# peter-nebe/stair-step-detector

Measured on AMD Instinct MI355X. Metric: point-cloud frames/sec (1024×768 pts) at 1/2/4/8 GPUs; step height/corner max-abs err, higher is better.
Workload: dtype f64; 1 GPU; BASELINE configs[2]: batch of 1024 synthetic 1024x768 frames (3-step staircases, randomised rise/tread/yaw/noise) resident in HBM, streamed through the whole per-frame path; per GPU; width=1024, height=768, input=float3, risers=False, batches_in_flight=3, parallelism=frame-sharded x1, no collective

## Files before the change

stair-step-detector_amd/csrc/ssd_kernels.hip:

```cpp
#ifndef SSD_CAMERAS_TU
#define SSD_ENTRY(bounds, kernel, block) __global__ bounds void kernel
#define SSD_BYVAL(T) T
#else
#define SSD_ENTRY(bounds, kernel, block) __device__ __forceinline__ void block
#define SSD_BYVAL(T) const T &
#undef SSD_PHASE_TIMING
#undef SSD_COUNT
#endif
#include "ssd_device.h"
#include "ssd_math.h"
#include "ssd_quadtest.h"
#include "ssd_closing.h"
#include "ssd_bestline.h"
#include "ssd_sort.h"

namespace ssd
{

#include "ssd_phase.h"

#ifdef SSD_CHECKED
__device__ __noinline__ void ssd_chk_report(int site, unsigned long long idx, unsigned long long limit)
{
  printf("SSD_CHECK site %d index %llu limit %llu block (%u, %u) thread %u\n", site, idx, limit, blockIdx.x, blockIdx.y, threadIdx.x);
// ... 113 lines not shown
  if(SRC == kSrcF3Aligned && idx0 + kPts <= end)
  {
    const float4 *q = reinterpret_cast<const float4 *>(base + 3 * static_cast<size_t>(idx0));
    const float4 a = q[0], b = q[1], c = q[2];
    v[0] = F3{ a.x, a.y, a.z };
    v[1] = F3{ a.w, b.x, b.y };
    v[2] = F3{ b.z, b.w, c.x };
    v[3] = F3{ c.y, c.z, c.w };
    return;
  }
#pragma unroll
  for(int j = 0; j < kPts; j++)
  {
    const int idx = idx0 + j;
    v[j] = F3{ 0.0f, 0.0f, 0.0f };
    if(idx < end)
      v[j] = *reinterpret_cast<const F3 *>(base + 3 * static_cast<size_t>(idx));
  }
}

template<int SRC>
__device__ __forceinline__ void load_points_full(const float *__restrict__ base, int idx0, F3 (&v)[kPts])
{
  if(SRC == kSrcDepth16)
    return;
  if(SRC == kSrcF3Aligned)
  {
    const float4 *q = reinterpret_cast<const float4 *>(base + 3 * static_cast<size_t>(idx0));
#ifdef SSD_NT_LOADS
    typedef float f4v __attribute__((ext_vector_type(4)));
    const f4v *qv = reinterpret_cast<const f4v *>(q);
    const f4v av = __builtin_nontemporal_load(qv), bv = __builtin_nontemporal_load(qv + 1), cv = __builtin_nontemporal_load(qv + 2);
    const float4 a = make_float4(av.x, av.y, av.z, av.w), b = make_float4(bv.x, bv.y, bv.z, bv.w), c = make_float4(cv.x, cv.y, cv.z, cv.w);
#else
    const float4 a = q[0], b = q[1], c = q[2];
#endif
    v[0] = F3{ a.x, a.y, a.z };
    v[1] = F3{ a.w, b.x, b.y };
    v[2] = F3{ b.z, b.w, c.x };
    v[3] = F3{ c.y, c.z, c.w };
    return;
  }
#pragma unroll
  for(int j = 0; j < kPts; j++)
    v[j] = *reinterpret_cast<const F3 *>(base + 3 * static_cast<size_t>(idx0 + j));
}

template<int SRC>
__device__ __forceinline__ void load_points_clamped(const float *__restrict__ base, int idx0, int end, F3 (&v)[kPts])
{
  if(SRC == kSrcDepth16)
    return;
  if(SRC == kSrcF3Aligned)
  {
    load_points_full<SRC>(base, min(idx0, end - kPts), v);
    return;
  }
#pragma unroll
  for(int j = 0; j < kPts; j++)
    v[j] = *reinterpret_cast<const F3 *>(base + 3 * static_cast<size_t>(min(idx0 + j, end - 1)));
}
__device__ __forceinline__ void zero_beyond(F3 (&v)[kPts], int idx0, int end)
{
#pragma unroll
  for(int j = 0; j < kPts; j++)
    if(idx0 + j >= end)
      v[j] = F3{ 0.0f, 0.0f, 0.0f };
}

__device__ __forceinline__ void first_use(F3 (&v)[kPts])
{
  asm volatile("" : "+v"(v[0].x), "+v"(v[0].y), "+v"(v[0].z), "+v"(v[1].x), "+v"(v[1].y), "+v"(v[1].z),
                    "+v"(v[2].x), "+v"(v[2].y), "+v"(v[2].z), "+v"(v[3].x), "+v"(v[3].y), "+v"(v[3].z));
}

#define SSD_STREAM_LOOP(body)                                                                       \
  {                                                                                                 \
    F3 va[kPts], vb[kPts];                                                                          \
    const int fullEnd = begin + (end - begin) / kTile * kTile;   \
    if(begin < fullEnd)                                                                             \
      load_points_full<SRC>(base, begin + kPts * tid, va);                                          \
    for(int i0 = begin; i0 < fullEnd; i0 += 2 * kTile)                                              \
    {                                                                                               \
      const bool more1 = i0 + kTile < fullEnd;                                                      \
      if(more1)                                                                                     \
        load_points_full<SRC>(base, i0 + kTile + kPts * tid, vb);                                   \
      body(va);                                                                                     \
      if(!more1)                                                                                    \
        break;                                                                                      \
      first_use(vb);                                                                                \
      const bool more2 = i0 + 2 * kTile < fullEnd;                                                  \
      if(more2)                                                                                     \
        load_points_full<SRC>(base, i0 + 2 * kTile + kPts * tid, va);                               \
      body(vb);                                                                                     \
      if(more2)                                                                                     \
        first_use(va);                                                                              \
    }                                                                                               \
    if(fullEnd < end)                                                                               \
    {                                                                                               \
      load_points<SRC>(base, fullEnd + kPts * tid, end, va, D);        \
      body(va);                                                                                     \
    }                                                                                               \
  }

constexpr int kBinsPerGroup = 4;
constexpr int kWavesPerBlock = kThreads / 64;
constexpr int kCell = 64;
constexpr int kCellsPerTile = kTile / kCell;
#ifndef SSD_MAX_TILES
#define SSD_MAX_TILES 32
#endif
constexpr int kMaxTilesPerBlock = SSD_MAX_TILES;
constexpr int kMaxCellsPerBlock = kMaxTilesPerBlock * kCellsPerTile;
constexpr int kMaxTilesPerBlockRaster = 128;
constexpr int kMaxCellsPerBlockRaster = kMaxTilesPerBlockRaster * kCellsPerTile;
constexpr int kMaxTilesPerBlockInquad = 128;
constexpr int kMaxCellsPerBlockInquad = kMaxTilesPerBlockInquad * kCellsPerTile;

__device__ __forceinline__ unsigned int row_or_u32(unsigned int v)
{
  v |= static_cast<unsigned int>(__builtin_amdgcn_update_dpp(0, static_cast<int>(v), 0x128, 0xf, 0xf, false));
  v |= static_cast<unsigned int>(__builtin_amdgcn_update_dpp(0, static_cast<int>(v), 0x124, 0xf, 0xf, false));
  v |= static_cast<unsigned int>(__builtin_amdgcn_update_dpp(0, static_cast<int>(v), 0x122, 0xf, 0xf, false));
  v |= static_cast<unsigned int>(__builtin_amdgcn_update_dpp(0, static_cast<int>(v), 0x121, 0xf, 0xf, false));
  return v;
}

__device__ __forceinline__ unsigned int row_min_u32(unsigned int v)
{
  v = min(v, static_cast<unsigned int>(__builtin_amdgcn_update_dpp(0, static_cast<int>(v), 0x128, 0xf, 0xf, false)));
  v = min(v, static_cast<unsigned int>(__builtin_amdgcn_update_dpp(0, static_cast<int>(v), 0x124, 0xf, 0xf, false)));
  v = min(v, static_cast<unsigned int>(__builtin_amdgcn_update_dpp(0, static_cast<int>(v), 0x122, 0xf, 0xf, false)));
  v = min(v, static_cast<unsigned int>(__builtin_amdgcn_update_dpp(0, static_cast<int>(v), 0x121, 0xf, 0xf, false)));
  return v;
}
__device__ __forceinline__ unsigned int row_max_u32(unsigned int v)
{
  v = max(v, static_cast<unsigned int>(__builtin_amdgcn_update_dpp(0, static_cast<int>(v), 0x128, 0xf, 0xf, false)));
  v = max(v, static_cast<unsigned int>(__builtin_amdgcn_update_dpp(0, static_cast<int>(v), 0x124, 0xf, 0xf, false)));
  v = max(v, static_cast<unsigned int>(__builtin_amdgcn_update_dpp(0, static_cast<int>(v), 0x122, 0xf, 0xf, false)));
  v = max(v, static_cast<unsigned int>(__builtin_amdgcn_update_dpp(0, static_cast<int>(v), 0x121, 0xf, 0xf, false)));
  return v;
}
__device__ __forceinline__ unsigned int cell_box_from_high_dwords(unsigned int x0, unsigned int x1, unsigned int y0, unsigned int y1,
                                                                  double boxX, double boxY)
{
  const unsigned int cx0 = static_cast<unsigned int>(__hiloint2double(static_cast<int>(x0), 0) * boxX);
  const unsigned int cy0 = static_cast<unsigned int>(__hiloint2double(static_cast<int>(y0), 0) * boxY);
  const unsigned int cx1 = min(static_cast<unsigned int>(__hiloint2double(static_cast<int>(x1 + 1u), 0) * boxX), 255u);
  const unsigned int cy1 = min(static_cast<unsigned int>(__hiloint2double(static_cast<int>(y1 + 1u), 0) * boxY), 255u);
  return (cx0 | (cx1 << 8)) | ((cy0 | (cy1 << 8)) << 16);
}

template<typename Want>
__device__ __forceinline__ int cell_list_build(const uint2 *__restrict__ cellInfo, int nCells, int cols, Want wantCell,
                                               unsigned short *list, unsigned int *scratch)
{
  const int tid = threadIdx.x, lane = tid & 63, wave = tid >> 6;
  const int rows = (nCells + cols - 1) / cols;
  constexpr int kFastPasses = 2;
  if(rows * cols <= kFastPasses * kThreads)
  {
    int cidx[kFastPasses];
    uint2 rec[kFastPasses];
#pragma unroll
    for(int p = 0; p < kFastPasses; p++)
    {
      const int i = p * kThreads + tid;
      const int cx = i / rows, r = i - cx * rows;
      const int c = r * cols + cx;
      cidx[p] = (cx < cols && c < nCells) ? c : -1;
      rec[p] = cidx[p] >= 0 ? cellInfo[c] : make_uint2(0u, 0u);
    }
    bool want[kFastPasses];
    int pos[kFastPasses];
#pragma unroll
    for(int p = 0; p < kFastPasses; p++)
    {
      want[p] = cidx[p] >= 0 && wantCell(rec[p]);
      const unsigned long long b = __ballot(want[p]);
      pos[p] = __popcll(b & ((1ull << lane) - 1ull));
      if(lane == 0)
        scratch[p * kWavesPerBlock + wave] = static_cast<unsigned int>(__popcll(b));
    }
    __syncthreads();
    int total = 0;
#pragma unroll
    for(int p = 0; p < kFastPasses; p++)
    {
      int before = total;
#pragma unroll
      for(int w = 0; w < kWavesPerBlock; w++)
      {
        const int n = static_cast<int>(scratch[p * kWavesPerBlock + w]);
        before += w < wave ? n : 0;
        total += n;
      }
      if(want[p])
        list[before + pos[p]] = static_cast<unsigned short>(cidx[p]);
    }
    __syncthreads();
    return total;
  }
  int total = 0;
  for(int i0 = 0; i0 < rows * cols; i0 += kThreads)
  {
    const int i = i0 + tid;
    const int cx = i / rows, r = i - cx * rows;
    const int c = r * cols + cx;
    const bool want = cx < cols && c < nCells && wantCell(cellInfo[c]);
    const unsigned long long b = __ballot(want);
    if(lane == 0)
      scratch[wave] = static_cast<unsigned int>(__popcll(b));
    __syncthreads();
    int before = total;
#pragma unroll
    for(int w = 0; w < kWavesPerBlock; w++)
    {
      const int n = static_cast<int>(scratch[w]);
      before += w < wave ? n : 0;
      total += n;
    }
    if(want)
      list[before + __popcll(b & ((1ull << lane) - 1ull))] = static_cast<unsigned short>(c);
    __syncthreads();
  }
  return total;
}

template<int SRC>
__device__ __forceinline__ void load_cell(const float *__restrict__ base, int cell0, const unsigned short *list, int entry, int count,
                                          int lane, int nPoints, F3 (&v)[kPts], const DepthSrc &D)
{
  if(entry < count)
    load_points<SRC>(base, (cell0 + static_cast<int>(list[entry])) * kCell + kPts * (lane & 15), nPoints, v, D);
  else
  {
#pragma unroll
    for(int j = 0; j < kPts; j++)
      v[j] = F3{ 0.0f, 0.0f, 0.0f };
  }
}


constexpr int kWinWords = 256;

struct ImageBox { int yMin, yMax, xMin, xMax; };

struct WaveWindow
{
  int slot = -1, row0 = 0, col0 = 0;
  unsigned int limitWords = 0xffffffffu;
};

constexpr int kWaveMissWords = 8;
__device__ __forceinline__ void wavemiss_init(unsigned int *wm)
{
  wm[0] = 0xffffffffu; wm[1] = 0u;
  wm[2] = 0x7fffffffu; wm[3] = 0xffffffffu;
  wm[4] = 0x7fffffffu; wm[5] = 0xffffffffu;
  wm[6] = 0u; wm[7] = 0u;
}
__device__ __forceinline__ void wavemiss_flush(unsigned int *wm, ImageBox *boxes, int lane)
{
  const unsigned int slots = wm[6];
  if(lane < 32 && ((slots >> lane) & 1u))
  {
    const int *b = reinterpret_cast<const int *>(wm);
    atomicMin(&boxes[lane].yMin, b[2]); atomicMax(&boxes[lane].yMax, b[3]);
    atomicMin(&boxes[lane].xMin, b[4]); atomicMax(&boxes[lane].xMax, b[5]);
  }
}

__device__ __forceinline__ int wave_min_i(int v)
{
  v = min(v, __builtin_amdgcn_update_dpp(0x7fffffff, v, 0x128, 0xf, 0xf, false));
  v = min(v, __builtin_amdgcn_update_dpp(0x7fffffff, v, 0x124, 0xf, 0xf, false));
  v = min(v, __builtin_amdgcn_update_dpp(0x7fffffff, v, 0x122, 0xf, 0xf, false));
  v = min(v, __builtin_amdgcn_update_dpp(0x7fffffff, v, 0x121, 0xf, 0xf, false));
  return min(min(__builtin_amdgcn_readlane(v, 0), __builtin_amdgcn_readlane(v, 16)), min(__builtin_amdgcn_readlane(v, 32), __builtin_amdgcn_readlane(v, 48)));
}
__device__ __forceinline__ int wave_max_i(int v)
{
  v = max(v, __builtin_amdgcn_update_dpp(static_cast<int>(0x80000000u), v, 0x128, 0xf, 0xf, false));
  v = max(v, __builtin_amdgcn_update_dpp(static_cast<int>(0x80000000u), v, 0x124, 0xf, 0xf, false));
  v = max(v, __builtin_amdgcn_update_dpp(static_cast<int>(0x80000000u), v, 0x122, 0xf, 0xf, false));
  v = max(v, __builtin_amdgcn_update_dpp(static_cast<int>(0x80000000u), v, 0x121, 0xf, 0xf, false));
  return max(max(__builtin_amdgcn_readlane(v, 0), __builtin_amdgcn_readlane(v, 16)), max(__builtin_amdgcn_readlane(v, 32), __builtin_amdgcn_readlane(v, 48)));
}

__device__ __forceinline__ void wavewin_flush(unsigned long long *ww, const WaveWindow &w, unsigned long long *__restrict__ images,
                                              unsigned int imgWords, int W64, int winShift, ImageBox *boxes, int lane)
{
  if(w.slot < 0)
    return;
  unsigned long long *img = images + static_cast<size_t>(w.slot) * imgWords;
  int y0 = 0x7fffffff, y1 = -1, x0 = 0x7fffffff, x1 = -1;
#pragma unroll
  for(int k = 0; k < kWinWords / 64; k++)
  {
    const int i = k * 64 + lane;
    const unsigned long long v = ww[i];
    if(v)
    {
      const int y = w.row0 + (i >> winShift), x = w.col0 + (i & ((1 << winShift) - 1));
      if(SSD_CHK(1, static_cast<size_t>(w.slot) * imgWords + static_cast<size_t>(y) * W64 + x, w.limitWords) && SSD_CHK(2, x, W64))
        atomicOr(img + static_cast<size_t>(y) * W64 + x, v);
      ww[i] = 0ull;
      y0 = min(y0, y); y1 = max(y1, y);
      x0 = min(x0, x); x1 = max(x1, x);
    }
  }
  y1 = wave_max_i(y1);
  if(y1 >= 0)
  {
    y0 = wave_min_i(y0); x0 = wave_min_i(x0); x1 = wave_max_i(x1);
    if(lane == 0)
    {
      atomicMin(&boxes[w.slot].yMin, y0); atomicMax(&boxes[w.slot].yMax, y1);
      atomicMin(&boxes[w.slot].xMin, x0); atomicMax(&boxes[w.slot].xMax, x1);
    }
  }
}

constexpr unsigned int kNoPixel = 0xffffffffu;
__device__ __forceinline__ unsigned int pixel_key(int slot, int iy, int ix)
{
  return (static_cast<unsigned int>(slot) << 26) | (static_cast<unsigned int>(iy) << 13) | static_cast<unsigned int>(ix);
}

__device__ __forceinline__ unsigned int wave_min_u32(unsigned int v)
{
  v = row_min_u32(v);
  return min(min(static_cast<unsigned int>(__builtin_amdgcn_readlane(static_cast<int>(v), 0)), static_cast<unsigned int>(__builtin_amdgcn_readlane(static_cast<int>(v), 16))),
             min(static_cast<unsigned int>(__builtin_amdgcn_readlane(static_cast<int>(v), 32)), static_cast<unsigned int>(__builtin_amdgcn_readlane(static_cast<int>(v), 48))));
}

constexpr unsigned int kNoWindow = 0x80000000u;
__device__ __forceinline__ unsigned int window_base(const WaveWindow &w)
{
  return w.slot < 0 ? kNoWindow : pixel_key(w.slot, w.row0, w.col0 << 6);
}
__device__ __forceinline__ bool window_hit(unsigned int d, int winShift)
{
  const unsigned int inside = (((static_cast<unsigned int>(kWinWords) >> winShift) - 1u) << 13) | ((64u << winShift) - 1u);
  return (d & ~inside) == 0u;
}

__device__ __forceinline__ void wavewin_prepare(unsigned long long *ww, WaveWindow &w, unsigned long long *__restrict__ images,
                                                unsigned int imgWords, int W64, int winShift, ImageBox *boxes, unsigned int first, int lane)
{
  const bool has = first != kNoPixel;
  const bool miss = has && !window_hit(first - window_base(w), winShift);
  const unsigned long long missing = __ballot(miss);
  if(missing == 0ull || 2 * __popcll(missing) <= __popcll(__ballot(has)))
    return;
  const unsigned int lowest = __builtin_amdgcn_readfirstlane(wave_min_u32(miss ? first : kNoPixel));
  wavewin_flush(ww, w, images, imgWords, W64, winShift, boxes, lane);
  w.slot = static_cast<int>(lowest >> 26);
  w.row0 = static_cast<int>((lowest >> 13) & 0x1fffu);
  w.col0 = max(0, min(static_cast<int>((lowest & 0x1fffu) >> 6) - 1, W64 - (1 << winShift)));
}

__device__ __forceinline__ void wavewin_emit(unsigned long long *ww, unsigned int *wm, WaveWindow &w, unsigned long long *__restrict__ images,
                                             unsigned int imgWords, int W64, int winShift, ImageBox *boxes, const unsigned int (&key)[4], int lane)
{
  wavewin_prepare(ww, w, images, imgWords, W64, winShift, boxes, min(min(key[0], key[1]), min(key[2], key[3])), lane);
  const unsigned int base = window_base(w);
  unsigned int *ww32 = reinterpret_cast<unsigned int *>(ww);
#pragma unroll
  for(int j = 0; j < 4; j++)
  {
    const unsigned int k = key[j], d = k - base;
    const unsigned int bit = 1u << (k & 31u);
    if(window_hit(d, winShift))
    {
      if(SSD_CHK(3, ((d >> 13) << (winShift + 1)) + ((d & 0x1fffu) >> 5), 2 * kWinWords))
        atomicOr(&ww32[((d >> 13) << (winShift + 1)) + ((d & 0x1fffu) >> 5)], bit);
    }
    else if(k != kNoPixel)
// ... 2028 lines not shown
    QuadTest t;
    SSD_PHASE_IF(lane == firstValid, 1, 3);
    build_quad_test(quad, t);
    err = t.err;
    SSD_PHASE_IF(lane == firstValid, 1, 4);
    const bool threwHere = __ballot(err != 0) != 0ull;
    const unsigned long long liveMask = threwHere ? 0ull : __ballot(true);
    if(!threwHere)
    {
      const int slot = __popcll(liveMask & ((1ull << lane) - 1ull));
      if(slot < kMaxLive)
      {
        fs.qtLive[slot] = t;
        QuadGridSegs sg;
        build_grid_segs(t, P.pt.xMin, P.pt.yMin, P.pt.boxX, P.pt.boxY, sg);
        fs.segLive[slot] = sg;
        QuadEdgesD w;
        quad_edges_coeffs(t, sg.ok, P.pt.xMin, P.pt.xMax, P.pt.yMin, P.pt.yMax, w, ef);
        sT[slot] = t;
        sW[slot] = w;
        sBad[slot] = 0u;
        mySlot = slot;
        fs.liveBox[slot] = live_box_thresholds(t, groundLane, P.pt);
        fs.liveAcc[slot] = static_cast<unsigned char>(lane);
        const PlateauState &pl = fs.pl[groundLane ? groundInd : lane];
        unsigned int groups = 0u;
        const int effLo = pl.effLo, effHi = pl.effHi;
        for(int b = effLo; b <= effHi; b++)
          groups |= 1u << (b / kBinsPerGroup);
        fs.liveGroups[slot] = groups;
      }
    }
  }
  {
    const int nL = __popcll(__ballot(mySlot >= 0));
    __syncthreads();
    for(int item = lane; item < nL * 9; item += 64)
    {
      const int sl = item / 9, cell = item - 9 * sl;
      if(sW[sl].fine != 0 && quad_cell_unsound(sT[sl], sW[sl], cell / 3, cell % 3))
        atomicOr(&sBad[sl], 1u);
    }
    __syncthreads();
    if(mySlot >= 0)
    {
      ef.m = quad_edges_margin(sW[mySlot], sBad[mySlot] != 0u);
      fs.edgeLive[mySlot] = ef;
    }
  }
  SSD_PHASE_IF(lane == firstValid, 1, 5);
  const bool threw = __ballot(err != 0) != 0ull;
  const bool active = (groundLane || valid) && !threw;
  if(lane <= kMaxPlateaus)
    fs.accActive[lane] = active ? 1 : 0;
  const unsigned long long activeMask = __ballot(active);
  for(int b = lane; b < kMaxBins; b += 64)
  {
    const int p = b < P.nBins ? fs.lut[b] : 0xff;
    const int acc = p == groundInd ? kGroundAcc : p;
    const bool live = p != 0xff && ((activeMask >> acc) & 1ull);
    fs.lutLive[b] = live ? static_cast<unsigned char>(__popcll(activeMask & ((1ull << acc) - 1ull))) : static_cast<unsigned char>(0xff);
  }

  SSD_PHASE_IF(lane == firstValid, 1, 6);
  unsigned int wanted = 0u;
  for(int b = lane; b < P.nBins; b += 64)
  {
    const int p = fs.lut[b];
    if(p != 0xff && ((activeMask >> (p == groundInd ? kGroundAcc : p)) & 1ull))
      wanted |= 1u << (b / kBinsPerGroup);
  }
#pragma unroll
  for(int o = 32; o > 0; o >>= 1)
    wanted |= __shfl_xor(wanted, o);
  if(lane == 0)
  {
    fs.firstValidInd = firstValid;
    if(threw)
      fs.status |= SSD_ST_THROW;
    fs.wantedQuads = wanted;
    fs.anyActive = activeMask != 0ull ? 1u : 0u;
    fs.nLive = min(__popcll(activeMask), kMaxLive);
  }
  SSD_PHASE_IF(lane == firstValid, 1, 7);
  if(dbg)
  {
    ssd_debug_frame &d = dbg[frame].d;
    if(lane == 0)
      d.first_valid_ind = firstValid;
    if(lane == kGroundAcc)
    {
      for(int k = 0; k < 8; k++)
        d.ground_quad_world[k] = groundLane ? fs.groundQuadWorld[k] : 0.0;
      d.ground_quad_err = groundLane ? err : 0;
    }
    if(lane >= first && lane < last && lane < kMaxPlateaus)
      d.plateaus[lane].quad_err = valid ? err : 0;
  }
}


constexpr int kGroundScanStep = 50;
__device__ __forceinline__ int ground_scan_x0(int W) { return (W / 2) % kGroundScanStep; }
__device__ __forceinline__ int ground_strip_row0(int H) { return H / 2 - 1; }
constexpr unsigned int strip_div50(unsigned int u) { return (u * 5243u) >> 18; }
constexpr bool strip_div50_exact()
{
  for(unsigned int u = 0; u < 16384u; u++)
    if(strip_div50(u) != u / 50u)
      return false;
  return true;
}
static_assert(strip_div50_exact(), "strip_div50 must equal u / 50 for every pixel column of an image up to 8192 wide");
__device__ __forceinline__ bool ground_strip_column(int ix, int x0)
{
  const unsigned int u = static_cast<unsigned int>(ix + 2 - x0 + kGroundScanStep);
  const unsigned int r = u - kGroundScanStep * strip_div50(u);
  return r <= 4u;
}
__device__ __forceinline__ bool ground_strip_of(int ix, int x0, int &strip, bool &centre)
{
  const unsigned int u = static_cast<unsigned int>(ix + 2 - x0 + kGroundScanStep);
  const unsigned int q = strip_div50(u), r = u - kGroundScanStep * q;
  strip = static_cast<int>(q);
  centre = r == 2u;
  return r <= 4u;
}
static_assert((8191 + 2 + kGroundScanStep) / kGroundScanStep < kMaxGroundStrips, "a strip number for every pixel column");

template<bool FULL>
struct InquadLds
{
  unsigned long long wins[FULL ? kThreads / 64 : 1][FULL ? kWinWords : 1];
  unsigned int wmiss[FULL ? kThreads / 64 : 1][kWaveMissWords];
  ImageBox box[1];
  QuadTest qts[kMaxLive];
  QuadGridSegs segs[kMaxLive];
  QuadEdgesF edges[kMaxLive + 1];
  K1Consts kc;
  unsigned char lut[kMaxBins];
  unsigned long long lsum[kMaxLive][8];
  unsigned int lcnt[kMaxLive][8];
  unsigned int lOob;
  unsigned short cellList[kMaxCellsPerBlockInquad];
  unsigned int listScratch[2 * kWavesPerBlock];
  unsigned int liveGroups[kMaxLive];
  int4 liveBox[kMaxLive];
  unsigned char liveAcc[kMaxLive];
  int nLive, groundSlot;
  int nextGroup;
  int stripMax[kMaxGroundStrips];
};

template<bool CHECKS, bool LABELS>
__device__ __forceinline__ void quad_decide(const F3 &p, const PreXY &Q, const PreLane lc, const QuadEdgesF *edges,
                                            const unsigned char *lut, const QuadTest *qts, const K1Consts &kc,
                                            const int gSlot, f32x2 &dOut, float &MOut, float &M3Out, unsigned int &qOut,
                                            unsigned long long &mSlowOut, unsigned long long &mCountOut, unsigned long long &mGroundOut)
{
  const PreRange r = pre_range<CHECKS, LABELS>(p, Q, lc);
  const float M3 = r.M3;
  f32x2 d = r.d;
  unsigned long long mSlow = r.mSlow;
  unsigned int q = kMaxLive;
  if(__builtin_amdgcn_inverse_ballot_w64(r.mInSure))
    q = SSD_CHK(28, r.b, kMaxBins) ? lut[r.b] : kMaxLive;
  const unsigned long long mLive = __ballot(q != static_cast<unsigned int>(kMaxLive));
  const QuadEdgesF &E = edges[q];
  const float4 gx = *reinterpret_cast<const float4 *>(E.gx), gy = *reinterpret_cast<const float4 *>(E.gy), g2 = *reinterpret_cast<const float4 *>(E.g2);
  f32x2 e01 = __builtin_elementwise_fma(f32x2{ gx.x, gx.y }, f32x2{ d.x, d.x }, f32x2{ g2.x, g2.y });
  f32x2 e23 = __builtin_elementwise_fma(f32x2{ gx.z, gx.w }, f32x2{ d.x, d.x }, f32x2{ g2.z, g2.w });
  e01 = __builtin_elementwise_fma(f32x2{ gy.x, gy.y }, f32x2{ d.y, d.y }, e01);
  e23 = __builtin_elementwise_fma(f32x2{ gy.z, gy.w }, f32x2{ d.y, d.y }, e23);
  const float emin = min3_f32(e01.x, e01.y, min_f32(e23.x, e23.y));
  const float hq = __builtin_fmaf(M3, Q.dK, E.m);
#if defined(SSD_SABOTAGE_PRE) && (SSD_SABOTAGE_PRE & 4)
  const unsigned long long mSureQ = mLive;
#elif defined(SSD_SABOTAGE_PRE) && (SSD_SABOTAGE_PRE & 32)
  const unsigned long long mSureQ = LABELS ? mLive : __ballot(__builtin_fabsf(emin) > hq);
#else
  const unsigned long long mSureQ = __ballot(__builtin_fabsf(emin) > hq);
#endif
  const unsigned long long mOutQ = __ballot(emin < 0.0f);
  unsigned long long mGround = __ballot(q == static_cast<unsigned int>(gSlot));
  unsigned long long mCount = mSureQ & (LABELS ? ~mOutQ : (mGround ^ mOutQ));
  mSlow |= mLive & ~mSureQ;
  if(__builtin_expect(mSlow != 0ull, 0))
  {
    const K1ConstsLds c = k1_consts(kc);
    const World3 w = world_rows(c, p);
    const bool mine = __builtin_amdgcn_inverse_ballot_w64(mSlow);
    const bool inRange = world_in_range(c, w);
    unsigned int qD = kMaxLive;
    bool counts = false;
    if(mine && inRange)
    {
      const int bD = world_bin(c, w);
      qD = SSD_CHK(29, bD, kMaxBins) ? lut[bD] : kMaxLive;
      if(qD != static_cast<unsigned int>(kMaxLive))
      {
        const QuadTest &tq = qts[qD];
        const bool fast = w.x >= tq.fx0 && w.x < tq.fx1 && w.y >= tq.fy0 && w.y < tq.fy1;
        const bool inside = fast || quad_test(tq, w.x, w.y);
        counts = LABELS ? inside : inside == (qD == static_cast<unsigned int>(gSlot));
      }
    }
    mCount = (mCount & ~mSlow) | __ballot(counts);
    mGround = (mGround & ~mSlow) | __ballot(qD == static_cast<unsigned int>(gSlot));
    q = mine ? qD : q;
    d.x = mine ? d_from_world(c, w).x : d.x;
    d.y = mine ? d_from_world(c, w).y : d.y;
  }
  dOut = d; MOut = r.M; M3Out = M3; qOut = q;
  mSlowOut = mSlow; mCountOut = mCount; mGroundOut = mGround;
}

template<int SRC, bool FULL, bool CHECKS>
__device__ __forceinline__ void inquad_block(InquadLds<FULL> &L, const float *__restrict__ xyz, size_t strideFloats, const PointParams &P,
                                             const PreXY &Q, const PixelParams &X, FrameState *__restrict__ st,
                                             unsigned long long *__restrict__ groundImg,
                                             const uint2 *__restrict__ tileMasks, size_t tileMaskStride, int chunkPoints, const DepthSrc &D,
                                             const int frame, const int chunkIdx)
{
  auto &wins = L.wins;
  auto &wmiss = L.wmiss;
  ImageBox (&box)[1] = L.box;
  QuadTest (&qts)[kMaxLive] = L.qts;
  QuadGridSegs (&segs)[kMaxLive] = L.segs;
  unsigned char (&lut)[kMaxBins] = L.lut;
  unsigned long long (&lsum)[kMaxLive][8] = L.lsum;
  unsigned int (&lcnt)[kMaxLive][8] = L.lcnt;
  unsigned int &lOob = L.lOob;
  unsigned short (&cellList)[kMaxCellsPerBlockInquad] = L.cellList;
  unsigned int (&listScratch)[2 * kWavesPerBlock] = L.listScratch;
  unsigned int (&liveGroups)[kMaxLive] = L.liveGroups;
  int4 (&liveBox)[kMaxLive] = L.liveBox;
  unsigned char (&liveAcc)[kMaxLive] = L.liveAcc;
  int &nLive = L.nLive;
  int &groundSlot = L.groundSlot;

  const int tid = threadIdx.x, lane = tid & 63;
  FrameState &fs = st[frame];
  const unsigned int anyActive = fs.anyActive;
  const unsigned char lutMine = tid < kMaxBins ? fs.lutLive[tid] : static_cast<unsigned char>(0xff);
  const unsigned char accMine = tid < kMaxLive ? fs.liveAcc[tid] : static_cast<unsigned char>(0);
  const unsigned int groupsMine = tid < kMaxLive ? fs.liveGroups[tid] : 0u;
  const int stripMaxMine = (!FULL && tid < kMaxGroundStrips) ? fs.groundStripMax[tid] : -1;
  const int4 boxMine = tid < kMaxLive ? fs.liveBox[tid] : make_int4(0, 0, 0, 0);
  const int nLiveG = fs.nLive;
  const unsigned char groundActive = fs.accActive[kGroundAcc];
  constexpr int qtWords = kMaxLive * static_cast<int>(sizeof(QuadTest) / 4), sgWords = kMaxLive * static_cast<int>(sizeof(QuadGridSegs) / 4);
  constexpr int qtPer = (qtWords + kThreads - 1) / kThreads, sgPer = (sgWords + kThreads - 1) / kThreads;
  unsigned int qtw[qtPer], sgw[sgPer];
  constexpr int egWords = kMaxLive * static_cast<int>(sizeof(QuadEdgesF) / 4);
  static_assert(sizeof(QuadEdgesF) == 64 && egWords + 16 <= 2 * kThreads, "two words of the edge table per thread");
  float edgeMine[2];
#pragma unroll
  for(int k = 0; k < 2; k++)
    edgeMine[k] = tid + k * kThreads < egWords ? reinterpret_cast<const float *>(fs.edgeLive)[tid + k * kThreads] : 0.0f;
  {
    const unsigned int *src = reinterpret_cast<const unsigned int *>(fs.qtLive);
    const unsigned int *srcS = reinterpret_cast<const unsigned int *>(fs.segLive);
#pragma unroll
    for(int k = 0; k < qtPer; k++)
      qtw[k] = tid + k * kThreads < qtWords ? src[tid + k * kThreads] : 0u;
#pragma unroll
    for(int k = 0; k < sgPer; k++)
      sgw[k] = tid + k * kThreads < sgWords ? srcS[tid + k * kThreads] : 0u;
  }
  if(!anyActive)
    return;
  BlockPhase ph(1);
  if(tid == 0)
  {
    box[0] = ImageBox{ 0x7fffffff, -1, 0x7fffffff, -1 };
    lOob = 0;
    nLive = nLiveG;
    groundSlot = (nLiveG > 0 && groundActive) ? nLiveG - 1 : -1;
    L.nextGroup = 0;
    k1_consts_fill(L.kc, P, &X);
  }
  if(tid < kMaxBins)
    lut[tid] = lutMine == 0xff ? static_cast<unsigned char>(kMaxLive) : lutMine;
#pragma unroll
  for(int k = 0; k < 2; k++)
  {
    const int w = tid + k * kThreads;
    if(w < egWords + 16)
      reinterpret_cast<float *>(L.edges)[w] = quad_edge_word(w, egWords, edgeMine[k], Q.dE0);
  }
  if(!FULL && tid < kMaxGroundStrips)
    L.stripMax[tid] = stripMaxMine;
  if(tid < kMaxLive)
  {
    liveAcc[tid] = accMine;
    liveGroups[tid] = groupsMine;
    liveBox[tid] = boxMine;
  }
  for(int i = tid; i < kMaxLive * 8; i += kThreads)
  {
    (&lsum[0][0])[i] = 0ull;
    (&lcnt[0][0])[i] = 0u;
  }
  if(FULL)
  {
    for(int i = tid; i < (kThreads / 64) * kWinWords; i += kThreads)
      (&wins[0][0])[i] = 0ull;
    if(tid < kThreads / 64)
      wavemiss_init(wmiss[tid]);
  }
  {
    unsigned int *dst = reinterpret_cast<unsigned int *>(qts);
    unsigned int *dstS = reinterpret_cast<unsigned int *>(segs);
#pragma unroll
    for(int k = 0; k < qtPer; k++)
      if(tid + k * kThreads < qtWords)
        dst[tid + k * kThreads] = qtw[k];
#pragma unroll
    for(int k = 0; k < sgPer; k++)
      if(tid + k * kThreads < sgWords)
        dstS[tid + k * kThreads] = sgw[k];
  }
  __syncthreads();
  ph.mark(0);

  const float *base = SRC == kSrcDepth16
    ? reinterpret_cast<const float *>(reinterpret_cast<const unsigned short *>(xyz) + static_cast<size_t>(frame) * strideFloats)
    : xyz + static_cast<size_t>(frame) * strideFloats;
  const int begin = chunkIdx * chunkPoints;
  const int end = min(begin + chunkPoints, P.nPoints);
  unsigned long long *gimg = groundImg + static_cast<size_t>(frame) * X.H * X.W64;
  const int copy = lane & 7;
  const unsigned int imgWords = static_cast<unsigned int>(X.H) * X.W64;
  unsigned long long *ww = wins[FULL ? tid >> 6 : 0];
  unsigned int *wm = wmiss[FULL ? tid >> 6 : 0];
  WaveWindow win;
  win.limitWords = imgWords;
  const int stripX0 = ground_scan_x0(X.W), stripRow0 = ground_strip_row0(X.H);
  int gy0 = 0x7fffffff, gy1 = -1;
  unsigned int *gimg32 = reinterpret_cast<unsigned int *>(gimg);

  int curQ = -1;
  unsigned long long accZ = 0;
  unsigned int accN = 0, oob = 0;
  auto flushAcc = [&]()
  {
    if(curQ >= 0 && accN)
    {
      atomicAdd(&lsum[curQ][copy], accZ - static_cast<unsigned long long>(accN) * static_cast<unsigned long long>(kMagicBits));
      atomicAdd(&lcnt[curQ][copy], accN);
    }
  };

  const int cell0 = begin / kCell;
  const int nCells = (end - begin + kCell - 1) / kCell;
  const unsigned int wantedQuads = fs.wantedQuads;
  const int gSlot = groundSlot;
  const int count = cell_list_build(tileMasks + static_cast<size_t>(frame) * tileMaskStride + cell0, nCells, X.cellCols,
                                    [&](const uint2 info)
                                    {
                                      if((info.x & wantedQuads) == 0u)
                                        return false;
                                      const int x0 = info.y & 0xffu, x1 = (info.y >> 8) & 0xffu, y0 = (info.y >> 16) & 0xffu, y1 = info.y >> 24;
                                      bool need = false;
                                      for(int q = 0; q < nLive; q++)
                                      {
                                        if((info.x & liveGroups[q]) == 0u)
                                          continue;
                                        const int4 b = liveBox[q];
                                        if(q == gSlot)
                                          need = need || !(x1 <= b.x || x0 >= b.y || y1 <= b.z || y0 >= b.w);
                                        else
                                        {
                                          const bool in = (x0 >= b.x && x1 <= b.y && y0 >= b.z && y1 <= b.w) || grid_box_inside(segs[q], x0, x1, y0, y1);
                                          need = need || !in;
                                        }
                                      }
                                      return need;
                                    }, cellList, listScratch);
  ph.mark(1);
  const int nGroups = (count + 3) >> 2;
  auto grab = [&]()
  {
    int v = 0;
    if(lane == 0)
      v = atomicAdd(&L.nextGroup, 1);
    return __builtin_amdgcn_readfirstlane(v);
  };
  int g = grab();
  F3 v[kPts], vn[kPts];
  const PreLane lc(Q);
  const float pixBorder = 0.5f - 2.0f / static_cast<float>(min(X.W, X.H));
  const float pixRowThr = 0.5f - static_cast<float>(stripRow0 - 1) / static_cast<float>(X.H);
  const float pixColA = static_cast<float>(X.W) * 0.02f;
  const float pixColB = (0.5f * static_cast<float>(X.W) + static_cast<float>(2 - stripX0 + kGroundScanStep) - 2.5f) * 0.02f + 0.5f;
  if(g < nGroups)
    load_cell<SRC>(base, cell0, cellList, 4 * g + (lane >> 4), count, lane, P.nPoints, v, D);
  while(g < nGroups)
  {
    const int gNext = grab();
    if(gNext < nGroups)
      load_cell<SRC>(base, cell0, cellList, 4 * gNext + (lane >> 4), count, lane, P.nPoints, vn, D);
    unsigned int key[kPts];
    #pragma unroll
    for(int j = 0; j < kPts; j++)
    {
      key[j] = kNoPixel;
      const F3 p{ v[j].x, v[j].y, v[j].z };
      f32x2 d;
      float M, M3;
      unsigned int q;
      unsigned long long mSlow, mCount, mGround;
      quad_decide<CHECKS, false>(p, Q, lc, L.edges, lut, qts, L.kc, gSlot, d, M, M3, q, mSlow, mCount, mGround);
      if(__builtin_amdgcn_inverse_ballot_w64(mCount))
      {
        double wz = (P.a[6] * static_cast<double>(p.x) + P.a[7] * static_cast<double>(p.y)) + P.a[8] * static_cast<double>(p.z);
        wz = wz + P.b[2];
        if(static_cast<int>(q) != curQ)
        {
          flushAcc();
          curQ = static_cast<int>(q); accZ = 0; accN = 0;
        }
        accZ += static_cast<unsigned long long>(z_plus_magic_bits(wz));
        accN++;
      }
      unsigned long long mPixel = mCount & mGround;
      if(!FULL)
      {
        const unsigned long long mBorder = __ballot(M > pixBorder);
        const unsigned long long mRow = __ballot(d.y <= pixRowThr);
        const float gc = __builtin_amdgcn_fractf(__builtin_fmaf(d.x, pixColA, pixColB)) - 0.5f;
        const unsigned long long mCol = __ballot(__builtin_fabsf(gc) < 0.07f);
        mPixel &= mSlow | mBorder | (mRow & mCol);
      }
      if(FULL ? mPixel != 0ull : __builtin_expect(mPixel != 0ull, 0))
      {
        if(__builtin_amdgcn_inverse_ballot_w64(mPixel))
        {
          int ix, iy;
          const bool inside = pre_pixel(p, d, M3, X, L.kc, ix, iy);
          oob += inside ? 0u : 1u;
          if(FULL)
            key[j] = inside ? pixel_key(0, iy, ix) : kNoPixel;
          else if(inside && iy >= stripRow0)
          {
            int strip;
            bool centre;
            if(ground_strip_of(ix, stripX0, strip, centre))
            {
              const int seen = SSD_CHK(24, strip, kMaxGroundStrips) ? L.stripMax[strip] : 0x7fffffff;
              if(iy >= seen - 2)
              {
                if(SSD_CHK(23, static_cast<unsigned int>(iy) * (2u * X.W64) + (static_cast<unsigned int>(ix) >> 5), 2u * static_cast<unsigned int>(X.H) * X.W64))
                  atomicOr(gimg32 + (static_cast<unsigned int>(iy) * (2u * X.W64) + (static_cast<unsigned int>(ix) >> 5)), 1u << (ix & 31));
                gy0 = min(gy0, iy);
                gy1 = max(gy1, iy);
                if(centre && iy > seen)
                  atomicMax(&L.stripMax[strip], iy);
              }
            }
          }
        }
      }
    }
    if(FULL)
      wavewin_emit(ww, wm, win, gimg, imgWords, X.W64, X.winShiftGround, box, key, lane);
    g = gNext;
#pragma unroll
    for(int j = 0; j < kPts; j++)
      v[j] = vn[j];
  }
  if(FULL)
  {
    wavewin_flush(ww, win, gimg, imgWords, X.W64, X.winShiftGround, box, lane);
    wavemiss_flush(wm, box, lane);
  }
  else
  {
    gy1 = wave_max_i(gy1);
    if(gy1 >= 0)
    {
      gy0 = wave_min_i(gy0);
      if(lane == 0)
      {
        atomicMin(&box[0].yMin, gy0); atomicMax(&box[0].yMax, gy1);
        atomicMin(&box[0].xMin, 0); atomicMax(&box[0].xMax, X.W64 - 1);
      }
    }
  }
  ph.mark(2);
  flushAcc();
  if(oob)
    atomicAdd(&lOob, oob);
  __syncthreads();
  if(!FULL && tid < kMaxGroundStrips && L.stripMax[tid] > stripMaxMine)
    atomicMax(&fs.groundStripMax[tid], L.stripMax[tid]);
  ph.mark(3);
  if(tid < nLive)
  {
    unsigned long long s = 0;
    unsigned int c = 0;
    for(int k = 0; k < 8; k++)
    {
      s += lsum[tid][k];
      c += lcnt[tid][k];
    }
    if(c)
    {
      const int acc = liveAcc[tid];
      atomicAdd(reinterpret_cast<unsigned long long *>(&fs.sumZ[acc]), s);
      atomicAdd(&fs.cnt[acc], c);
    }
  }
  if(tid == 0)
  {
    if(box[0].yMax >= 0)
    {
      atomicMin(&fs.imgYMin[kMaxStepImages], box[0].yMin); atomicMax(&fs.imgYMax[kMaxStepImages], box[0].yMax);
      atomicMin(&fs.imgXMin[kMaxStepImages], box[0].xMin); atomicMax(&fs.imgXMax[kMaxStepImages], box[0].xMax);
    }
    if(lOob)
    {
      atomicAdd(&fs.nOob, lOob);
      atomicOr(&fs.status, static_cast<unsigned int>(SSD_ST_OOB_PIXEL));
    }
  }
  ph.mark(4);
  ph.finish();
}

#ifndef SSD_CAMERAS_TU
template<int SRC, bool FULL, bool CHECKS>
__global__ __launch_bounds__(kThreads, FULL ? 4 : SSD_K4_WAVES) void k_inquad(const float *__restrict__ xyz, size_t strideFloats, PointParams P, PreXY Q,
                                                        PixelParams X, FrameState *__restrict__ st,
                                                        unsigned long long *__restrict__ groundImg,
                                                        const uint2 *__restrict__ tileMasks, size_t tileMaskStride, int chunkPoints, DepthSrc D)
{
  __shared__ InquadLds<FULL> L;
  const int nChunks = static_cast<int>(gridDim.y), first = max(1, nChunks / 8), by = static_cast<int>(blockIdx.y);
  const int chunkIdx = by < first ? nChunks - 1 - by : by - first;
  inquad_block<SRC, FULL, CHECKS>(L, xyz, strideFloats, P, Q, X, st, groundImg, tileMasks, tileMaskStride, chunkPoints, D, blockIdx.x, chunkIdx);
}
#endif


struct LabelsLds
{
  QuadTest qts[kMaxLive];
  QuadEdgesF edges[kMaxLive + 1];
  K1Consts kc;
  unsigned char lut[kMaxBins];
  unsigned char label[kMaxLive + 1];
  unsigned short cellList[kMaxCellsPerBlock];
  unsigned int listScratch[2 * kWavesPerBlock];
};

__device__ __forceinline__ void store_labels4(unsigned char *__restrict__ row, bool aligned4, int idx, int nPoints, unsigned int word)
{
  if(aligned4 && idx + 4 <= nPoints)
    *reinterpret_cast<unsigned int *>(row + idx) = word;
  else
  {
#pragma unroll
    for(int k = 0; k < 4; k++)
      if(idx + k < nPoints)
        row[idx + k] = static_cast<unsigned char>(word >> (8 * k));
  }
}

template<int SRC, bool CHECKS>
SSD_ENTRY(__launch_bounds__(kThreads), k_labels, labels_block)(const float *__restrict__ xyz, size_t strideFloats, SSD_BYVAL(PointParams) P, SSD_BYVAL(PreXY) Q,
                                                     const FrameState *__restrict__ st, const uint2 *__restrict__ tileMasks,
                                                     size_t tileMaskStride, int chunkPoints, SSD_BYVAL(DepthSrc) D,
                                                     unsigned char *__restrict__ labels, size_t labelStride)
{
  __shared__ LabelsLds L;
  const int tid = threadIdx.x, lane = tid & 63;
  const int frame = blockIdx.x;
  const FrameState &fs = st[frame];
  const bool live = fs.anyActive != 0u && (fs.status & SSD_ST_THROW) == 0u;
  const unsigned int wanted = live ? fs.wantedQuads : 0u;
  if(live)
  {
    const int nLive = fs.nLive;
    const int gSlot = (nLive > 0 && fs.accActive[kGroundAcc]) ? nLive - 1 : -1;
    if(tid < kMaxBins)
    {
      const unsigned char s = fs.lutLive[tid];
      L.lut[tid] = s == 0xff ? static_cast<unsigned char>(kMaxLive) : s;
    }
    if(tid <= kMaxLive)
    {
      int lab = 0;
      if(tid < nLive)
        lab = tid == gSlot ? 1 : tid + 1 + (gSlot >= 0 ? 1 : 0);
      L.label[tid] = static_cast<unsigned char>(lab <= SSD_MAX_STEPS ? lab : 0);
    }
    constexpr int qtWords = kMaxLive * static_cast<int>(sizeof(QuadTest) / 4);
    constexpr int egWords = kMaxLive * static_cast<int>(sizeof(QuadEdgesF) / 4);
    for(int w = tid; w < qtWords; w += kThreads)
      reinterpret_cast<unsigned int *>(L.qts)[w] = reinterpret_cast<const unsigned int *>(fs.qtLive)[w];
    stage_quad_edges(L.edges, fs.edgeLive, egWords, Q.dE0);
    if(tid == 0)
    {
      K1Consts &c = L.kc;
      for(int i = 0; i < 9; i++)
        c.a[i] = P.a[i];
      c.b[0] = P.b[0]; c.b[1] = P.b[1]; c.b[2] = P.b[2];
      c.xMin = P.xMin; c.xMax = P.xMax; c.yMin = P.yMin; c.yMax = P.yMax; c.zMin = P.zMin; c.zMax = P.zMax;
      c.boxX = P.boxX; c.boxY = P.boxY;
      c.recip = P.recip;
      c.xToImage = 0.0; c.yToImage = 0.0;
    }
  }
  __syncthreads();

  const float *base = SRC == kSrcDepth16
    ? reinterpret_cast<const float *>(reinterpret_cast<const unsigned short *>(xyz) + static_cast<size_t>(frame) * strideFloats)
    : xyz + static_cast<size_t>(frame) * strideFloats;
  unsigned char *row = labels + static_cast<size_t>(frame) * labelStride;
  const int begin = blockIdx.y * chunkPoints;
  const int end = min(begin + chunkPoints, P.nPoints);
  const int cell0 = begin / kCell;
// ... 732 lines not shown
```

Measured before the change: 378,600 frames/s.

## Split inquad cell list into general and ground-interior classes with lean decide path

The cell list builder now sorts cells into two classes: general cells, and cells lying fully inside the ground quad's grid interior. The interior class is walked with a lean quad_decide that skips the per-point edge-plane tests and sure/out ballots. The aim is to cut per-point ALU and LDS work for the bulk of ground points in the non-FULL path. In exchange it adds a second ballot and prefix sum during list building, kNoCell padding, and two instantiations of the walk loop. Correctness depends on the interior classification being conservative.

Result: slower. 370,900 frames/s (-2.0%).

```diff
diff --git a/stair-step-detector_amd/csrc/ssd_kernels.hip b/stair-step-detector_amd/csrc/ssd_kernels.hip
--- a/stair-step-detector_amd/csrc/ssd_kernels.hip
+++ b/stair-step-detector_amd/csrc/ssd_kernels.hip
@@ -289,13 +289,15 @@
   return (cx0 | (cx1 << 8)) | ((cy0 | (cy1 << 8)) << 16);
 }
 
-template<typename Want>
-__device__ __forceinline__ int cell_list_build(const uint2 *__restrict__ cellInfo, int nCells, int cols, Want wantCell,
-                                               unsigned short *list, unsigned int *scratch)
+constexpr unsigned short kNoCell = 0xffff;
+template<bool TWO, typename Class>
+__device__ __forceinline__ int cell_list_build_classes(const uint2 *__restrict__ cellInfo, int nCells, int cols, Class classOf,
+                                                       unsigned short *list, unsigned int *scratch, int &countSecond)
 {
   const int tid = threadIdx.x, lane = tid & 63, wave = tid >> 6;
   const int rows = (nCells + cols - 1) / cols;
   constexpr int kFastPasses = 2;
+  countSecond = 0;
   if(rows * cols <= kFastPasses * kThreads)
   {
     int cidx[kFastPasses];
@@ -309,32 +311,64 @@
       cidx[p] = (cx < cols && c < nCells) ? c : -1;
       rec[p] = cidx[p] >= 0 ? cellInfo[c] : make_uint2(0u, 0u);
     }
-    bool want[kFastPasses];
-    int pos[kFastPasses];
+    bool want[kFastPasses], second[kFastPasses];
+    int pos[kFastPasses], posSecond[kFastPasses];
 #pragma unroll
     for(int p = 0; p < kFastPasses; p++)
     {
-      want[p] = cidx[p] >= 0 && wantCell(rec[p]);
+      const int cls = cidx[p] >= 0 ? static_cast<int>(classOf(rec[p])) : 0;
+      want[p] = cls == 1;
+      second[p] = TWO && cls == 2;
       const unsigned long long b = __ballot(want[p]);
       pos[p] = __popcll(b & ((1ull << lane) - 1ull));
+      unsigned int n = static_cast<unsigned int>(__popcll(b));
+      posSecond[p] = 0;
+      if constexpr(TWO)
+      {
+        const unsigned long long b2 = __ballot(second[p]);
+        posSecond[p] = __popcll(b2 & ((1ull << lane) - 1ull));
+        n |= static_cast<unsigned int>(__popcll(b2)) << 16;
+      }
       if(lane == 0)
-        scratch[p * kWavesPerBlock + wave] = static_cast<unsigned int>(__popcll(b));
+        scratch[p * kWavesPerBlock + wave] = n;
     }
     __syncthreads();
-    int total = 0;
+    int total = 0, totalSecond = 0;
+    int before[kFastPasses], beforeSecond[kFastPasses];
 #pragma unroll
     for(int p = 0; p < kFastPasses; p++)
     {
-      int before = total;
+      before[p] = total;
+      beforeSecond[p] = totalSecond;
 #pragma unroll
       for(int w = 0; w < kWavesPerBlock; w++)
       {
-        const int n = static_cast<int>(scratch[p * kWavesPerBlock + w]);
-        before += w < wave ? n : 0;
+        const unsigned int nn = scratch[p * kWavesPerBlock + w];
+        const int n = static_cast<int>(TWO ? nn & 0xffffu : nn);
+        before[p] += w < wave ? n : 0;
         total += n;
+        if constexpr(TWO)
+        {
+          const int n2 = static_cast<int>(nn >> 16);
+          beforeSecond[p] += w < wave ? n2 : 0;
+          totalSecond += n2;
+        }
       }
       if(want[p])
-        list[before + pos[p]] = static_cast<unsigned short>(cidx[p]);
+        list[before[p] + pos[p]] = static_cast<unsigned short>(cidx[p]);
+    }
+    if constexpr(TWO)
+    {
+      const int start = (total + 3) & ~3, end = start + totalSecond;
+#pragma unroll
+      for(int p = 0; p < kFastPasses; p++)
+        if(second[p])
+          list[start + beforeSecond[p] + posSecond[p]] = static_cast<unsigned short>(cidx[p]);
+      if(tid < 3 && total + tid < start)
+        list[total + tid] = kNoCell;
+      if(tid < 3 && end + tid < ((end + 3) & ~3))
+        list[end + tid] = kNoCell;
+      countSecond = totalSecond;
     }
     __syncthreads();
     return total;
@@ -345,7 +379,7 @@
     const int i = i0 + tid;
     const int cx = i / rows, r = i - cx * rows;
     const int c = r * cols + cx;
-    const bool want = cx < cols && c < nCells && wantCell(cellInfo[c]);
+    const bool want = cx < cols && c < nCells && classOf(cellInfo[c]) != 0;
     const unsigned long long b = __ballot(want);
     if(lane == 0)
       scratch[wave] = static_cast<unsigned int>(__popcll(b));
@@ -362,7 +396,20 @@
       list[before + __popcll(b & ((1ull << lane) - 1ull))] = static_cast<unsigned short>(c);
     __syncthreads();
   }
+  if constexpr(TWO)
+  {
+    if(tid < 3 && total + tid < ((total + 3) & ~3))
+      list[total + tid] = kNoCell;
+    __syncthreads();
+  }
   return total;
+}
+template<typename Want>
+__device__ __forceinline__ int cell_list_build(const uint2 *__restrict__ cellInfo, int nCells, int cols, Want wantCell,
+                                               unsigned short *list, unsigned int *scratch)
+{
+  int none;
+  return cell_list_build_classes<false>(cellInfo, nCells, cols, [&](const uint2 info) { return wantCell(info) ? 1 : 0; }, list, scratch, none);
 }
 
 template<int SRC>
@@ -2697,7 +2744,7 @@
   int stripMax[kMaxGroundStrips];
 };
 
-template<bool CHECKS, bool LABELS>
+template<bool CHECKS, bool LABELS, bool LEAN = false>
 __device__ __forceinline__ void quad_decide(const F3 &p, const PreXY &Q, const PreLane lc, const QuadEdgesF *edges,
                                             const unsigned char *lut, const QuadTest *qts, const K1Consts &kc,
                                             const int gSlot, f32x2 &dOut, float &MOut, float &M3Out, unsigned int &qOut,
@@ -2710,26 +2757,30 @@
   unsigned int q = kMaxLive;
   if(__builtin_amdgcn_inverse_ballot_w64(r.mInSure))
     q = SSD_CHK(28, r.b, kMaxBins) ? lut[r.b] : kMaxLive;
-  const unsigned long long mLive = __ballot(q != static_cast<unsigned int>(kMaxLive));
-  const QuadEdgesF &E = edges[q];
-  const float4 gx = *reinterpret_cast<const float4 *>(E.gx), gy = *reinterpret_cast<const float4 *>(E.gy), g2 = *reinterpret_cast<const float4 *>(E.g2);
-  f32x2 e01 = __builtin_elementwise_fma(f32x2{ gx.x, gx.y }, f32x2{ d.x, d.x }, f32x2{ g2.x, g2.y });
-  f32x2 e23 = __builtin_elementwise_fma(f32x2{ gx.z, gx.w }, f32x2{ d.x, d.x }, f32x2{ g2.z, g2.w });
-  e01 = __builtin_elementwise_fma(f32x2{ gy.x, gy.y }, f32x2{ d.y, d.y }, e01);
-  e23 = __builtin_elementwise_fma(f32x2{ gy.z, gy.w }, f32x2{ d.y, d.y }, e23);
-  const float emin = min3_f32(e01.x, e01.y, min_f32(e23.x, e23.y));
-  const float hq = __builtin_fmaf(M3, Q.dK, E.m);
+  unsigned long long mGround = __ballot(q == static_cast<unsigned int>(gSlot));
+  unsigned long long mCount = mGround;
+  if constexpr(!LEAN)
+  {
+    const unsigned long long mLive = __ballot(q != static_cast<unsigned int>(kMaxLive));
+    const QuadEdgesF &E = edges[q];
+    const float4 gx = *reinterpret_cast<const float4 *>(E.gx), gy = *reinterpret_cast<const float4 *>(E.gy), g2 = *reinterpret_cast<const float4 *>(E.g2);
+    f32x2 e01 = __builtin_elementwise_fma(f32x2{ gx.x, gx.y }, f32x2{ d.x, d.x }, f32x2{ g2.x, g2.y });
+    f32x2 e23 = __builtin_elementwise_fma(f32x2{ gx.z, gx.w }, f32x2{ d.x, d.x }, f32x2{ g2.z, g2.w });
+    e01 = __builtin_elementwise_fma(f32x2{ gy.x, gy.y }, f32x2{ d.y, d.y }, e01);
+    e23 = __builtin_elementwise_fma(f32x2{ gy.z, gy.w }, f32x2{ d.y, d.y }, e23);
+    const float emin = min3_f32(e01.x, e01.y, min_f32(e23.x, e23.y));
+    const float hq = __builtin_fmaf(M3, Q.dK, E.m);
 #if defined(SSD_SABOTAGE_PRE) && (SSD_SABOTAGE_PRE & 4)
-  const unsigned long long mSureQ = mLive;
+    const unsigned long long mSureQ = mLive;
 #elif defined(SSD_SABOTAGE_PRE) && (SSD_SABOTAGE_PRE & 32)
-  const unsigned long long mSureQ = LABELS ? mLive : __ballot(__builtin_fabsf(emin) > hq);
+    const unsigned long long mSureQ = LABELS ? mLive : __ballot(__builtin_fabsf(emin) > hq);
 #else
-  const unsigned long long mSureQ = __ballot(__builtin_fabsf(emin) > hq);
+    const unsigned long long mSureQ = __ballot(__builtin_fabsf(emin) > hq);
 #endif
-  const unsigned long long mOutQ = __ballot(emin < 0.0f);
-  unsigned long long mGround = __ballot(q == static_cast<unsigned int>(gSlot));
-  unsigned long long mCount = mSureQ & (LABELS ? ~mOutQ : (mGround ^ mOutQ));
-  mSlow |= mLive & ~mSureQ;
+    const unsigned long long mOutQ = __ballot(emin < 0.0f);
+    mCount = mSureQ & (LABELS ? ~mOutQ : (mGround ^ mOutQ));
+    mSlow |= mLive & ~mSureQ;
+  }
   if(__builtin_expect(mSlow != 0ull, 0))
   {
     const K1ConstsLds c = k1_consts(kc);
@@ -2759,6 +2810,8 @@
   dOut = d; MOut = r.M; M3Out = M3; qOut = q;
   mSlowOut = mSlow; mCountOut = mCount; mGroundOut = mGround;
 }
+
+template<bool B> struct BoolTag { static constexpr bool value = B; };
 
 template<int SRC, bool FULL, bool CHECKS>
 __device__ __forceinline__ void inquad_block(InquadLds<FULL> &L, const float *__restrict__ xyz, size_t strideFloats, const PointParams &P,
@@ -2901,13 +2954,25 @@
   const int nCells = (end - begin + kCell - 1) / kCell;
   const unsigned int wantedQuads = fs.wantedQuads;
   const int gSlot = groundSlot;
-  const int count = cell_list_build(tileMasks + static_cast<size_t>(frame) * tileMaskStride + cell0, nCells, X.cellCols,
+#ifdef SSD_K4_ONE_LIST
+  constexpr bool kTwoLists = false;
+#else
+  constexpr bool kTwoLists = !FULL && !CHECKS && SRC != kSrcDepth16;
+#endif
+  const bool groundLean = kTwoLists && gSlot >= 0 && L.edges[gSlot >= 0 ? gSlot : 0].m < INFINITY;
+#ifdef SSD_K4_INTERIOR_FIRST
+  constexpr int kGeneral = 2, kInterior = 1;
+#else
+  constexpr int kGeneral = 1, kInterior = 2;
+#endif
+  int countSecond = 0;
+  const int count = cell_list_build_classes<kTwoLists>(tileMasks + static_cast<size_t>(frame) * tileMaskStride + cell0, nCells, X.cellCols,
                                     [&](const uint2 info)
                                     {
                                       if((info.x & wantedQuads) == 0u)
-                                        return false;
+                                        return 0;
                                       const int x0 = info.y & 0xffu, x1 = (info.y >> 8) & 0xffu, y0 = (info.y >> 16) & 0xffu, y1 = info.y >> 24;
-                                      bool need = false;
+                                      bool need = false, lean = groundLean;
                                       for(int q = 0; q < nLive; q++)
                                       {
                                         if((info.x & liveGroups[q]) == 0u)
@@ -2919,12 +2984,37 @@
                                         {
                                           const bool in = (x0 >= b.x && x1 <= b.y && y0 >= b.z && y1 <= b.w) || grid_box_inside(segs[q], x0, x1, y0, y1);
                                           need = need || !in;
+                                          lean = false;
                                         }
                                       }
-                                      return need;
-                                    }, cellList, listScratch);
+                                      if(!need)
+                                        return 0;
+#ifdef SSD_SABOTAGE_K4_INTERIOR
+                                      return lean ? kInterior : kGeneral;
+#else
+                                      return lean && grid_box_inside(segs[gSlot], x0, x1, y0, y1) ? kInterior : kGeneral;
+#endif
+                                    }, cellList, listScratch, countSecond);
   ph.mark(1);
-  const int nGroups = (count + 3) >> 2;
+  const int nGroupsFirst = (count + 3) >> 2;
+  const int nGroups = nGroupsFirst + ((countSecond + 3) >> 2);
+  auto loadGroup = [&](const int gi, F3 (&dst)[kPts])
+  {
+    if constexpr(!kTwoLists)
+      load_cell<SRC>(base, cell0, cellList, 4 * gi + (lane >> 4), count, lane, P.nPoints, dst, D);
+    else
+    {
+      const unsigned int c = cellList[4 * gi + (lane >> 4)];
+      if(c != kNoCell)
+        load_points<SRC>(base, (cell0 + static_cast<int>(c)) * kCell + kPts * (lane & 15), P.nPoints, dst, D);
+      else
+      {
+#pragma unroll
+        for(int j = 0; j < kPts; j++)
+          dst[j] = F3{ 0.0f, 0.0f, 0.0f };
+      }
+    }
+  };
   auto grab = [&]()
   {
     int v = 0;
@@ -2940,80 +3030,91 @@
   const float pixColA = static_cast<float>(X.W) * 0.02f;
   const float pixColB = (0.5f * static_cast<float>(X.W) + static_cast<float>(2 - stripX0 + kGroundScanStep) - 2.5f) * 0.02f + 0.5f;
   if(g < nGroups)
-    load_cell<SRC>(base, cell0, cellList, 4 * g + (lane >> 4), count, lane, P.nPoints, v, D);
-  while(g < nGroups)
-  {
-    const int gNext = grab();
-    if(gNext < nGroups)
-      load_cell<SRC>(base, cell0, cellList, 4 * gNext + (lane >> 4), count, lane, P.nPoints, vn, D);
-    unsigned int key[kPts];
-    #pragma unroll
-    for(int j = 0; j < kPts; j++)
-    {
-      key[j] = kNoPixel;
-      const F3 p{ v[j].x, v[j].y, v[j].z };
-      f32x2 d;
-      float M, M3;
-      unsigned int q;
-      unsigned long long mSlow, mCount, mGround;
-      quad_decide<CHECKS, false>(p, Q, lc, L.edges, lut, qts, L.kc, gSlot, d, M, M3, q, mSlow, mCount, mGround);
-      if(__builtin_amdgcn_inverse_ballot_w64(mCount))
-      {
-        double wz = (P.a[6] * static_cast<double>(p.x) + P.a[7] * static_cast<double>(p.y)) + P.a[8] * static_cast<double>(p.z);
-        wz = wz + P.b[2];
-        if(static_cast<int>(q) != curQ)
+    loadGroup(g, v);
+  auto walk = [&](auto lean, const int gEnd)
+  {
+    constexpr bool LEAN = decltype(lean)::value;
+    while(g < gEnd)
+    {
+      const int gNext = grab();
+      if(gNext < nGroups)
+        loadGroup(gNext, vn);
+      unsigned int key[kPts];
+      #pragma unroll
+      for(int j = 0; j < kPts; j++)
+      {
+        key[j] = kNoPixel;
+        const F3 p{ v[j].x, v[j].y, v[j].z };
+        f32x2 d;
+        float M, M3;
+        unsigned int q;
+        unsigned long long mSlow, mCount, mGround;
+        quad_decide<CHECKS, false, LEAN>(p, Q, lc, L.edges, lut, qts, L.kc, gSlot, d, M, M3, q, mSlow, mCount, mGround);
+        if(__builtin_amdgcn_inverse_ballot_w64(mCount))
         {
-          flushAcc();
-          curQ = static_cast<int>(q); accZ = 0; accN = 0;
+          double wz = (P.a[6] * static_cast<double>(p.x) + P.a[7] * static_cast<double>(p.y)) + P.a[8] * static_cast<double>(p.z);
+          wz = wz + P.b[2];
+          if(static_cast<int>(q) != curQ)
+          {
+            flushAcc();
+            curQ = static_cast<int>(q); accZ = 0; accN = 0;
+          }
+          accZ += static_cast<unsigned long long>(z_plus_magic_bits(wz));
+          accN++;
         }
-        accZ += static_cast<unsigned long long>(z_plus_magic_bits(wz));
-        accN++;
-      }
-      unsigned long long mPixel = mCount & mGround;
-      if(!FULL)
-      {
-        const unsigned long long mBorder = __ballot(M > pixBorder);
-        const unsigned long long mRow = __ballot(d.y <= pixRowThr);
-        const float gc = __builtin_amdgcn_fractf(__builtin_fmaf(d.x, pixColA, pixColB)) - 0.5f;
-        const unsigned long long mCol = __ballot(__builtin_fabsf(gc) < 0.07f);
-        mPixel &= mSlow | mBorder | (mRow & mCol);
-      }
-      if(FULL ? mPixel != 0ull : __builtin_expect(mPixel != 0ull, 0))
-      {
-        if(__builtin_amdgcn_inverse_ballot_w64(mPixel))
+        unsigned long long mPixel = mCount & mGround;
+        if(!FULL)
         {
-          int ix, iy;
-          const bool inside = pre_pixel(p, d, M3, X, L.kc, ix, iy);
-          oob += inside ? 0u : 1u;
-          if(FULL)
-            key[j] = inside ? pixel_key(0, iy, ix) : kNoPixel;
-          else if(inside && iy >= stripRow0)
+          const unsigned long long mBorder = __ballot(M > pixBorder);
+          const unsigned long long mRow = __ballot(d.y <= pixRowThr);
+          const float gc = __builtin_amdgcn_fractf(__builtin_fmaf(d.x, pixColA, pixColB)) - 0.5f;
+          const unsigned long long mCol = __ballot(__builtin_fabsf(gc) < 0.07f);
+          mPixel &= mSlow | mBorder | (mRow & mCol);
+        }
+        if(FULL ? mPixel != 0ull : __builtin_expect(mPixel != 0ull, 0))
+        {
+          if(__builtin_amdgcn_inverse_ballot_w64(mPixel))
           {
-            int strip;
-            bool centre;
-            if(ground_strip_of(ix, stripX0, strip, centre))
+            int ix, iy;
+            const bool inside = pre_pixel(p, d, M3, X, L.kc, ix, iy);
+            oob += inside ? 0u : 1u;
+            if(FULL)
+              key[j] = inside ? pixel_key(0, iy, ix) : kNoPixel;
+            else if(inside && iy >= stripRow0)
             {
-              const int seen = SSD_CHK(24, strip, kMaxGroundStrips) ? L.stripMax[strip] : 0x7fffffff;
-              if(iy >= seen - 2)
+              int strip;
+              bool centre;
+              if(ground_strip_of(ix, stripX0, strip, centre))
               {
-                if(SSD_CHK(23, static_cast<unsigned int>(iy) * (2u * X.W64) + (static_cast<unsigned int>(ix) >> 5), 2u * static_cast<unsigned int>(X.H) * X.W64))
-                  atomicOr(gimg32 + (static_cast<unsigned int>(iy) * (2u * X.W64) + (static_cast<unsigned int>(ix) >> 5)), 1u << (ix & 31));
-                gy0 = min(gy0, iy);
-                gy1 = max(gy1, iy);
-                if(centre && iy > seen)
-                  atomicMax(&L.stripMax[strip], iy);
+                const int seen = SSD_CHK(24, strip, kMaxGroundStrips) ? L.stripMax[strip] : 0x7fffffff;
+                if(iy >= seen - 2)
+                {
+                  if(SSD_CHK(23, static_cast<unsigned int>(iy) * (2u * X.W64) + (static_cast<unsigned int>(ix) >> 5), 2u * static_cast<unsigned int>(X.H) * X.W64))
+                    atomicOr(gimg32 + (static_cast<unsigned int>(iy) * (2u * X.W64) + (static_cast<unsigned int>(ix) >> 5)), 1u << (ix & 31));
+                  gy0 = min(gy0, iy);
+                  gy1 = max(gy1, iy);
+                  if(centre && iy > seen)
+                    atomicMax(&L.stripMax[strip], iy);
+                }
               }
             }
           }
         }
       }
-    }
-    if(FULL)
-      wavewin_emit(ww, wm, win, gimg, imgWords, X.W64, X.winShiftGround, box, key, lane);
-    g = gNext;
-#pragma unroll
-    for(int j = 0; j < kPts; j++)
-      v[j] = vn[j];
+      if(FULL)
+        wavewin_emit(ww, wm, win, gimg, imgWords, X.W64, X.winShiftGround, box, key, lane);
+      g = gNext;
+#pragma unroll
+      for(int j = 0; j < kPts; j++)
+        v[j] = vn[j];
+    }
+  };
+  if constexpr(!kTwoLists)
+    walk(BoolTag<false>(), nGroups);
+  else
+  {
+    walk(BoolTag<kInterior == 1>(), nGroupsFirst);
+    walk(BoolTag<kInterior == 2>(), nGroups);
   }
   if(FULL)
   {
```
